# MaxInGaussian/SCFGP

Hardware: AMD Instinct MI355X
Metric: NLML+grad evals/sec (higher is better)
Workload: dtype f32

## Files before the change

scfgp_amd/csrc/apply.hip:

```cpp
#include "kernels.h"
#include "tile_cfgs.h"

#include <algorithm>

#ifdef SCFGP_TRACE
constexpr int ATRACE_CAP = 1 << 16;
__device__ unsigned long long g_atrace[5 * ATRACE_CAP][5];
int64_t apply_trace_read(void* host, int64_t max_bytes) {
    const int64_t n = max_bytes < (int64_t)sizeof(g_atrace) ? max_bytes : (int64_t)sizeof(g_atrace);
    return hipMemcpyFromSymbol(host, HIP_SYMBOL(g_atrace), n) == hipSuccess ? n : -2;
}
#else
int64_t apply_trace_read(void*, int64_t) { return -1; }
#endif
template <typename T, int TILE> struct ApplyCfg {
    typedef TileCfg<T, Tune<T>::APPLY_BM, TILE, SCFGP_BK, Tune<T>::APPLY_WGM, Tune<T>::apply_wgn(TILE), Tune<T>::MS,
                    SCFGP_BK == 16 && Tune<T>::MS == 16> type;
};

#include "apply_epilogue.h"

template <class Cfg, int EPI>
__device__ __forceinline__ void apply_tile(
    const typename Cfg::T* __restrict__ Phi, const typename Cfg::T* __restrict__ Bm, typename Cfg::T* V,
// ... 40 lines not shown
            __syncthreads();
            apply_tile<Cfg, EPI>(Phi, Bm, V, vpart, p, q, y, alpha, ut, K, Kp, Np, njt, col0, jt0, mu, ntot, o, rb, smem_raw);
        }
    } else
        apply_tile<Cfg, EPI>(Phi, Bm, V, vpart, p, q, y, alpha, ut, K, Kp, Np, njt, col0, jt0, mu, ntot, (int)(wid % njt), wid / njt, smem_raw);
}

typedef __attribute__((address_space(3))) void lds_void;
typedef const __attribute__((address_space(1))) void gbl_void;
template <typename T, int BN_>
struct ApplyDma {
    static constexpr int ES = (int)sizeof(T), BM = 256, BN = BN_, ROWB = 16 * ES, CPR = ROWB / 16;
    static constexpr int WN = ES == 4 ? 64 : 32;
    static constexpr int WAVES = 4 * (BN / WN), STAGE = (BM + BN) * ROWB, STAGES = 3, LDS_BYTES = STAGES * STAGE,
                         DMA_PER_WAVE = STAGE / 1024 / WAVES, ROWS_PER_DMA = 1024 / ROWB;
    static constexpr int PRE = 2;
    static constexpr int WAVES_PER_EU = WAVES == 4 ? 2 : 4;
    typedef TileCfg<T, BM, BN, 16, 4, BN / WN, 16, true> Cfg;
    static_assert(STAGE / 1024 % WAVES == 0 && LDS_BYTES <= 160 * 1024, "whole DMA instructions per wave; the ring fits the LDS");
    static __device__ __forceinline__ int swz(int x) {
        if constexpr (ES == 4) return (0x78 >> (2 * ((x >> 2) & 3))) & 3;
        else return (int)((0x6BEB08u >> (3 * ((x >> 1) & 7))) & 7);
    }
};
static_assert(((0x6BEB08u >> 0) & 7) == 0 && ((0x6BEB08u >> 3) & 7) == 1 && ((0x6BEB08u >> 6) & 7) == 4 && ((0x6BEB08u >> 9) & 7) == 5 &&
              ((0x6BEB08u >> 12) & 7) == 6 && ((0x6BEB08u >> 15) & 7) == 7 && ((0x6BEB08u >> 18) & 7) == 2 && ((0x6BEB08u >> 21) & 7) == 3,
              "fp64 swizzle table");

template <typename T, int EPI, int BN>
__global__ __launch_bounds__((64 * ApplyDma<T, BN>::WAVES)) __attribute__((amdgpu_waves_per_eu(ApplyDma<T, BN>::WAVES_PER_EU, ApplyDma<T, BN>::WAVES_PER_EU)))
void apply_dma_kernel(const T* __restrict__ Phi, const T* __restrict__ Bm, T* V,
                      double* __restrict__ vpart, const double* __restrict__ p, const double* __restrict__ q,
                      const double* __restrict__ y, const double* __restrict__ alpha, const double* __restrict__ ut,
                      int K, int Kp, int64_t Np, int njt, double* __restrict__ mu, int col0, int slot0, int64_t rb0) {
    typedef ApplyDma<T, BN> D;
    typedef typename D::Cfg Cfg;
    typedef T half_t __attribute__((ext_vector_type(2)));
    typedef std::integral_constant<int, 0> H0;
    typedef std::integral_constant<int, 1> H1;
    constexpr int DPW = D::DMA_PER_WAVE, NRD = Cfg::TM + Cfg::TN, NM = 2 * Cfg::TM * Cfg::TN, PRE = D::PRE;
    static_assert(Cfg::TM == 4 && (Cfg::TN == 4 || Cfg::TN == 2), "fragment lists of the wait statements");
    static_assert(PRE + DPW + NRD <= NM, "one fetch or read per MFMA behind the barrier");
    SMEM_DECL;
    char* smem = smem_raw;
#ifdef SCFGP_TRACE
    const unsigned long long tr_t0 = __builtin_amdgcn_s_memrealtime();
#endif
    const unsigned wid = xcd_remap(blockIdx.x, gridDim.x);
    const int jt = EPI == 3 || EPI == 4 ? (int)((wid % njt + wid / njt) % njt) : (int)(wid % njt);
    const int64_t rb = rb0 + wid / njt;
    const int cbase = col0 + jt * D::BN;
    const int lane = threadIdx.x & 63, wave = __builtin_amdgcn_readfirstlane(threadIdx.x >> 6);
    const char* src[DPW]; unsigned loff[DPW]; int dst[DPW];
#pragma unroll
    for (int u = 0; u < DPW; ++u) {
        const int t = wave * DPW + u, x0 = D::ROWS_PER_DMA * t, l = lane / D::CPR, c = (lane % D::CPR) ^ D::swz(x0 + l);
        const int xb = x0 - D::BM, xcol = (xb & ~(D::WN - 1)) + Cfg::TN * (xb & 15) + ((xb >> 4) & (Cfg::TN - 1));
        const T* rowp = x0 < D::BM ? Phi + (rb * D::BM + x0) * Kp : Bm + (int64_t)(cbase + xcol) * Kp;
        src[u] = reinterpret_cast<const char*>(rowp) + (EPI == 4 ? (cbase / 16) * D::ROWB : 0);
        loff[u] = (unsigned)((x0 < D::BM ? l : Cfg::TN * l) * Kp * D::ES + c * 16);
        dst[u] = t * 1024;
    }
    const auto fetch_one = [&](auto uc, int slot) {
        constexpr int u = decltype(uc)::value;
        __builtin_amdgcn_global_load_lds((gbl_void*)(src[u] + loff[u]), (lds_void*)(smem + slot * D::STAGE + dst[u]), 16, 0, 0);
        src[u] += D::ROWB;
    };
    const int i = lane & 15, qg = lane >> 4;
    const int wm0 = (wave / Cfg::WGN) * Cfg::WM, wn0 = (wave % Cfg::WGN) * Cfg::WN;
    const int hoff0 = sizeof(T) == 4 ? (((qg >> 1) ^ D::swz(i)) << 4) + 8 * (qg & 1) : ((2 * qg) ^ D::swz(i)) << 4;
    const int hoff1 = sizeof(T) == 4 ? (((2 + (qg >> 1)) ^ D::swz(i)) << 4) + 8 * (qg & 1) : ((2 * qg + 1) ^ D::swz(i)) << 4;
    const int ring = (int)(uintptr_t)smem, aoff = ring + (wm0 + i) * D::ROWB, boff = ring + D::BM * D::ROWB + (wn0 + i) * D::ROWB;
    const int ra[2] = {aoff + hoff0, aoff + hoff1}, rbb[2] = {boff + hoff0, boff + hoff1};
    half_t ha[2][Cfg::TM], hb[2][Cfg::TN];
    typename Cfg::MTr::acc_t acc[Cfg::TM][Cfg::TN];
    acc_zero<Cfg>(acc);
    const int nst_all = (K + 15) / 16, nst_tri = (cbase + D::BN + 15) / 16;
    const int nst = (EPI == 3 && nst_tri < nst_all ? nst_tri : nst_all) - (EPI == 4 ? cbase / 16 : 0);
#define SCFGP_LDS_READ(dst, addr, off)                                                                              \
    do {                                                                                                             \
        if constexpr (sizeof(T) == 4) asm volatile("ds_read_b64 %0, %1 offset:%2" : "=v"(dst) : "v"(addr), "n"(off));   \
// ... 118 lines not shown
template <typename T> struct ApplyPlan {
    static constexpr int NW = 2;
    int width[NW], count[NW], col0[NW], jt0[NW], total;
    explicit ApplyPlan(int K) {
        const int w[NW] = {128, 64};
        int col = 0, jt = 0;
        const bool small = K <= 256;
        for (int i = 0; i < NW; ++i) {
            width[i] = w[i];
            const bool last = i == NW - 1;
            count[i] = small && !last ? 0 : (last ? (K - col + w[i] - 1) / w[i] : (K - col) / w[i]);
            col0[i] = col; jt0[i] = jt;
            col += count[i] * w[i]; jt += count[i];
        }
        total = jt;
    }
};
bool F16x3Kernels::apply_runs(const Geom& g) { return ApplyPlan<float>(g.K).count[0] > 0; }
template <class Cfg, int EPI, typename T>
static int apply_launch_cfg(const Geom& g, int njt, int col0, int jt0, const T* Phi, const T* Bm, T* V, double* vpart,
                            const double* p, const double* q, const double* y, const double* alpha, const double* ut,
                            double* mu, int ntot, hipStream_t st) {
    if (njt <= 0) return 0;
    const int64_t nrb = g.Np / Cfg::BM;
    const int wgs_per_rb = EPI == 3 || EPI == 4 ? (njt + 1) / 2 : njt;
    allow_big_lds(apply_kernel<Cfg, EPI>, Cfg::LDS_BYTES);
    hipLaunchKernelGGL((apply_kernel<Cfg, EPI>), dim3((unsigned)(wgs_per_rb * nrb)), dim3(Cfg::THREADS), Cfg::LDS_BYTES, st,
                       Phi, Bm, V, vpart, p, q, y, alpha, ut, g.K, g.Kp, g.Np, njt, col0, jt0, mu, ntot);
    return (int)(njt * nrb);
}
template <typename T, int EPI, int BN>
static int apply_dma_launch(const Geom& g, int njt, int col0, int slot0, const T* Phi, const T* Bm, T* V, double* vpart,
                            const double* p, const double* q, const double* y, const double* alpha, const double* ut,
                            double* mu, hipStream_t st, int64_t rb0 = 0, int64_t nrb = -1) {
    typedef ApplyDma<T, BN> D;
    if (nrb < 0) nrb = g.Np / D::BM;
    if (njt <= 0 || nrb <= 0) return 0;
    allow_big_lds(apply_dma_kernel<T, EPI, BN>, D::LDS_BYTES);
    hipLaunchKernelGGL((apply_dma_kernel<T, EPI, BN>), dim3((unsigned)(njt * nrb)), dim3(64 * D::WAVES), D::LDS_BYTES, st,
                       Phi, Bm, V, vpart, p, q, y, alpha, ut, g.K, g.Kp, g.Np, njt, mu, col0, slot0, rb0);
    return (int)(njt * nrb);
}
static int apply_num_cus() {
    static int n = 0;
    if (n == 0) {
        int dev = 0; hipDeviceProp_t prop;
        if (hipGetDevice(&dev) == hipSuccess && hipGetDeviceProperties(&prop, dev) == hipSuccess) n = prop.multiProcessorCount;
        if (n <= 0) n = 256;
    }
    return n;
}
template <typename T, int EPI>
static int apply_launch(const Geom& g, const T* Phi, const T* Bm, T* V, double* vpart, const double* p, const double* q,
                        const double* y, const double* alpha, const double* ut, double* mu, hipStream_t st,
                        int dma = 0, const T* BmT = nullptr, const F16Operands* f16 = nullptr) {
    if (!BmT) BmT = Bm;
    const ApplyPlan<T> pl(g.K);
    int nb = 0;
    if constexpr (EPI != 2) {
        if (dma && pl.count[0] > 0) {
            int n256 = 0;
            const int64_t nrb = g.Np / 256;
            int64_t tail_rb = 0;
            if constexpr (sizeof(T) == 4) {
                n256 = dma == 2 ? pl.count[0] / 2 : 0;
                if (n256 > 0 && EPI != 3 && EPI != 4) {
                    const int64_t ncu = apply_num_cus(), tiles = nrb * n256, rem = tiles % ncu;
                    if (tiles > ncu && rem > 0 && 20 * rem <= 9 * ncu) tail_rb = (rem + n256 - 1) / n256;
                }
                if (f16 && (EPI == 0 || EPI == 1)) {
                    constexpr int E = EPI == 1 ? 1 : 0;
                    nb += F16x3Kernels::apply<E, 256>(g, n256, 0, 0, Phi, *f16, V, vpart, p, q, y, alpha, ut, mu, st, 0, nrb - tail_rb);
                    nb += F16x3Kernels::apply<E, 128>(g, pl.count[0] - 2 * n256, 256 * n256, 2 * n256, Phi, *f16, V, vpart, p, q, y, alpha, ut, mu, st, 0, nrb - tail_rb);
                    nb += F16x3Kernels::apply<E, 64>(g, pl.count[1], pl.col0[1], pl.jt0[1], Phi, *f16, V, vpart, p, q, y, alpha, ut, mu, st, 0, nrb - tail_rb);
                    if (tail_rb > 0) {
                        nb += F16x3Kernels::apply<E, 128>(g, pl.count[0], 0, 0, Phi, *f16, V, vpart, p, q, y, alpha, ut, mu, st, nrb - tail_rb, tail_rb);
                        nb += F16x3Kernels::apply<E, 64>(g, pl.count[1], pl.col0[1], pl.jt0[1], Phi, *f16, V, vpart, p, q, y, alpha, ut, mu, st, nrb - tail_rb, tail_rb);
                    }
                    return nb;
                }
                nb += apply_dma_launch<T, EPI, 256>(g, n256, 0, 0, Phi, BmT, V, vpart, p, q, y, alpha, ut, mu, st, 0, nrb - tail_rb);
            }
            nb += apply_dma_launch<T, EPI, 128>(g, pl.count[0] - 2 * n256, 256 * n256, 2 * n256, Phi, BmT, V, vpart, p, q, y, alpha, ut, mu, st, 0, nrb - tail_rb);
            nb += apply_dma_launch<T, EPI, 64>(g, pl.count[1], pl.col0[1], pl.jt0[1], Phi, BmT, V, vpart, p, q, y, alpha, ut, mu, st, 0, nrb - tail_rb);
            if (tail_rb > 0) {
                nb += apply_dma_launch<T, EPI, 128>(g, pl.count[0], 0, 0, Phi, BmT, V, vpart, p, q, y, alpha, ut, mu, st, nrb - tail_rb, tail_rb);
                nb += apply_dma_launch<T, EPI, 64>(g, pl.count[1], pl.col0[1], pl.jt0[1], Phi, BmT, V, vpart, p, q, y, alpha, ut, mu, st, nrb - tail_rb, tail_rb);
            }
            return nb;
        }
    }
    nb += apply_launch_cfg<typename ApplyCfg<T, 128>::type, EPI, T>(g, pl.count[0], pl.col0[0], pl.jt0[0], Phi, Bm, V, vpart, p, q, y, alpha, ut, mu, pl.total, st);
    nb += apply_launch_cfg<typename ApplyCfg<T, 64>::type, EPI, T>(g, pl.count[1], pl.col0[1], pl.jt0[1], Phi, Bm, V, vpart, p, q, y, alpha, ut, mu, pl.total, st);
    return nb;
}

template <typename T>
void ApplyKernels<T>::apply_v(const Geom& g, const T* Phi, const T* Bm, T* V, double* vpart, const double* alpha, double* mu,
                              hipStream_t st, int dma, const F16Operands* f16) {
    apply_launch<T, 0>(g, Phi, Bm, V, vpart, nullptr, nullptr, nullptr, alpha, nullptr, mu, st, dma, nullptr, f16);
}
template <typename T>
void ApplyKernels<T>::apply_predict(const Geom& g, const T* Phi, const T* LiT, double* vpart, const double* alpha, double* mu,
                                    hipStream_t st) {
    apply_launch<T, 2>(g, Phi, LiT, (T*)nullptr, vpart, nullptr, nullptr, nullptr, alpha, nullptr, mu, st);
}
template <typename T>
void ApplyKernels<T>::apply_plain(const Geom& g, const T* A, const T* Bm, T* Out, int Kc, int ncols, hipStream_t st) {
    Geom gk = g; gk.K = Kc;
    apply_launch_cfg<typename ApplyCfg<T, 64>::type, 4, T>(gk, (ncols + 63) / 64, 0, 0, A, Bm, Out, nullptr, nullptr, nullptr, nullptr, nullptr,
                                                           nullptr, nullptr, ApplyPlan<T>(Kc).total, st);
}

template <typename T>
void ApplyKernels<T>::apply_c(const Geom& g, const T* Phi, const T* LiT, const T* Li, T* C, double* vpart, const double* alpha,
                              const double* beta, double* mu, hipStream_t st, int dma) {
    const bool by_dma = dma && ApplyPlan<T>(g.K).count[0] > 0;
    apply_launch<T, 3>(g, Phi, LiT, C, vpart, nullptr, nullptr, nullptr, by_dma ? beta : alpha, nullptr, mu, st, dma, Li);
}
template <typename T>
void ApplyKernels<T>::apply_vc(const Geom& g, const T* C, const T* Li, const T* LiT, T* V, hipStream_t st, int dma) {
    apply_launch<T, 4>(g, C, Li, V, nullptr, nullptr, nullptr, nullptr, nullptr, nullptr, nullptr, st, dma, LiT);
}
template <typename T>
void ApplyKernels<T>::apply_phibar(const Geom& g, const T* Phi, const T* Abar, T* V, const double* p, const double* q,
                                   const double* y, const double* alpha, const double* ut, hipStream_t st, int dma, const F16Operands* f16) {
    apply_launch<T, 1>(g, Phi, Abar, V, nullptr, p, q, y, alpha, ut, nullptr, st, dma, nullptr, f16);
}

template <typename T> static int apply_njt(const Geom& g) { return ApplyPlan<T>(g.K).total; }


template <int MODE>
__global__ __launch_bounds__(256) void rowstats_kernel(const double* __restrict__ mupart, const double* __restrict__ vpart, int njt,
                                                       const double* __restrict__ y, const Scal* __restrict__ sc,
                                                       double* __restrict__ o1, double* __restrict__ o2,
                                                       double* __restrict__ partial, int64_t N, int64_t Np) {
    __shared__ double red[4][256];
    const double kappa = sc->kappa;
    double t2 = 0, kb = 0, qv = 0, pm = 0;
    for (int64_t n = (int64_t)blockIdx.x * 256 + threadIdx.x; n < Np; n += (int64_t)gridDim.x * 256) {
        double v = 0, mu = 0;
        for (int t = 0; t < njt; ++t) { v += vpart[(int64_t)t * Np + n]; mu += mupart[(int64_t)t * Np + n]; }
        const double d = kappa * (v + 1.0);
        if (MODE == 0) {
            double pn = 0, qn = 0;
            if (n < N) {
                const double r = mu - y[n];
                const double rv = r * r + v;
                const double e = 1.0 / d - rv / (d * d);
                pn = 2.0 * r / d;
                qn = 1.0 / d + kappa * e;
                t2 += rv / d + log(2.0 * M_PI * d);
                kb += e * (v + 1.0);
                qv += qn * v; pm += pn * mu;
            }
            o1[n] = pn; o2[n] = qn;
        } else if (n < N) {
            o1[n] = mu; o2[n] = sqrt(d);
        }
    }
    if (MODE == 0) {
        red[0][threadIdx.x] = t2; red[1][threadIdx.x] = kb; red[2][threadIdx.x] = qv; red[3][threadIdx.x] = pm;
        __syncthreads();
        for (int w = 128; w >= 1; w >>= 1) {
            if ((int)threadIdx.x < w)
                for (int k = 0; k < 4; ++k) red[k][threadIdx.x] += red[k][threadIdx.x + w];
            __syncthreads();
        }
        if (threadIdx.x < 4) partial[blockIdx.x * 4 + threadIdx.x] = red[threadIdx.x][0];
    }
}

template <typename T>
void ApplyKernels<T>::rowstats(const Geom& g, const double* mupart, const double* vpart, const double* y,
                               const Scal* sc, double* p, double* q, double* partial, int nblocks, hipStream_t st) {
    hipLaunchKernelGGL((rowstats_kernel<0>), dim3(nblocks), dim3(256), 0, st, mupart, vpart, apply_njt<T>(g), y, sc, p, q,
                       partial, g.N, g.Np);
}

template <typename T>
void ApplyKernels<T>::rowpredict(const Geom& g, const double* mupart, const double* vpart, const Scal* sc, double* mu, double* sd,
                                 hipStream_t st) {
    const int nblocks = (int)((g.Np + 255) / 256 < 1024 ? (g.Np + 255) / 256 : 1024);
    hipLaunchKernelGGL((rowstats_kernel<1>), dim3(nblocks), dim3(256), 0, st, mupart, vpart, apply_njt<T>(g),
                       (const double*)nullptr, sc, mu, sd, (double*)nullptr, g.N, g.Np);
}
template <typename T> int ApplyKernels<T>::partials(const Geom& g) { return apply_njt<T>(g); }
__global__ __launch_bounds__(256) void rowresidual_kernel(const double* __restrict__ mupart, int njt, const double* __restrict__ y,
                                                          double* __restrict__ r, int64_t N, int64_t Np) {
    for (int64_t n = (int64_t)blockIdx.x * 256 + threadIdx.x; n < Np; n += (int64_t)gridDim.x * 256) {
        double mu = 0;
        for (int t = 0; t < njt; ++t) mu += mupart[(int64_t)t * Np + n];
        r[n] = n < N ? y[n] - mu : 0.0;
    }
}
template <typename T>
void ApplyKernels<T>::rowresidual(const Geom& g, const double* mupart, const double* y, double* r, hipStream_t st) {
    const int nblocks = (int)((g.Np + 255) / 256 < 1024 ? (g.Np + 255) / 256 : 1024);
    hipLaunchKernelGGL(rowresidual_kernel, dim3(nblocks), dim3(256), 0, st, mupart, apply_njt<T>(g), y, r, g.N, g.Np);
}
template struct ApplyKernels<double>;
template struct ApplyKernels<float>;

__global__ __launch_bounds__(256) void reduce_scalars_kernel(const double* __restrict__ partial, int nblocks, int width,
                                                             double* __restrict__ scalars, int slot0) {
    __shared__ double red[256];
    for (int k = 0; k < width; ++k) {
        double s = 0;
        for (int b = threadIdx.x; b < nblocks; b += 256) s += partial[(int64_t)b * width + k];
        red[threadIdx.x] = s;
        __syncthreads();
        for (int m = 128; m >= 1; m >>= 1) {
            if (threadIdx.x < m) red[threadIdx.x] += red[threadIdx.x + m];
            __syncthreads();
        }
        if (threadIdx.x == 0) scalars[slot0 + k] = red[0];
        __syncthreads();
// ... 55 lines not shown
```

scfgp_amd/csrc/apply_f16.hip:

```cpp
#include "apply_epilogue.h"

typedef _Float16 h8 __attribute__((ext_vector_type(8)));
typedef _Float16 h4 __attribute__((ext_vector_type(4)));
typedef _Float16 h2 __attribute__((ext_vector_type(2)));
typedef __attribute__((address_space(3))) void lds_void;
typedef const __attribute__((address_space(1))) void gbl_void;

namespace {
constexpr int BM = 256, ROW = 128;
template <int BN_> struct F16Tile {
    static constexpr int BN = BN_, WAVES = 4 * (BN / 64), STAGE = (BM + BN) * ROW, STAGES = 2, LDS_BYTES = STAGES * STAGE,
                         DPW = STAGE / 1024 / WAVES, WAVES_PER_EU = WAVES == 16 ? 4 : 2;
    static_assert(STAGE / 1024 % WAVES == 0 && LDS_BYTES <= 160 * 1024, "whole DMA instructions per wave; the ring fits the LDS");
    typedef TileCfg<float, BM, BN, 16, 4, BN / 64, 16, true> Cfg;
};
__device__ __forceinline__ int swz8(int x) { return (int)((0x6BEB08u >> (3 * ((x >> 1) & 7))) & 7); }
template <int OFF> __device__ __forceinline__ void lds_read(h8& out, unsigned addr) {
    asm volatile("ds_read_b128 %0, %1 offset:%2" : "=v"(out) : "v"(addr), "n"(OFF));
}
#define SCFGP_F16_WAIT(n, x) asm volatile("s_waitcnt lgkmcnt(" #n ")" : "+v"(x[0]), "+v"(x[1]), "+v"(x[2]), "+v"(x[3]) :: "memory")
}

template <int EPI, int BN>
__global__ __launch_bounds__((64 * F16Tile<BN>::WAVES))
__attribute__((amdgpu_waves_per_eu(F16Tile<BN>::WAVES_PER_EU, F16Tile<BN>::WAVES_PER_EU)))
void apply_f16_kernel(const float* __restrict__ Phi, const unsigned* __restrict__ Phi16, const char* __restrict__ B16, const float* __restrict__ scale,
                      unsigned* __restrict__ V16, const float* __restrict__ vbound, float* V, double* __restrict__ vpart, const double* __restrict__ p, const double* __restrict__ q,
                      const double* __restrict__ y, const double* __restrict__ alpha, const double* __restrict__ ut,
                      int K, int Kp, int64_t Np, int njt, double* __restrict__ mu, int col0, int slot0, int64_t rb0) {
    typedef F16Tile<BN> D;
    typedef typename D::Cfg Cfg;
    constexpr int DPW = D::DPW, STAGE = D::STAGE;
    SMEM_DECL;
    char* smem = smem_raw;
    const unsigned wid = xcd_remap(blockIdx.x, gridDim.x);
    const int jt = wid % njt;
    const int64_t rb = rb0 + wid / njt;
    const int cbase = col0 + jt * BN;
    const int lane = threadIdx.x & 63, wave = __builtin_amdgcn_readfirstlane(threadIdx.x >> 6);
    const char* src[DPW]; int dst[DPW];
#pragma unroll
    for (int u = 0; u < DPW; ++u) {
        const int t = DPW * wave + u, x = 8 * t + lane / 8;
        if (x < BM) {
            src[u] = reinterpret_cast<const char*>(Phi16 + (rb * BM + x) * Kp) + (((lane % 8) ^ swz8(x)) << 4);
        } else {
            const int xb = x - BM, xcol = (xb & ~63) + 4 * (xb & 15) + ((xb >> 4) & 3);
            src[u] = B16 + (int64_t)(cbase + xcol) * Kp * 4 + (((lane % 8) ^ swz8(xb)) << 4);
        }
        dst[u] = t * 1024;
    }
    const auto fetch = [&](int slot) {
#pragma unroll
        for (int u = 0; u < DPW; ++u) {
            __builtin_amdgcn_global_load_lds((gbl_void*)src[u], (lds_void*)(smem + slot * STAGE + dst[u]), 16, 0, 0);
            src[u] += ROW;
        }
    };
    const int i = lane & 15, qg = lane >> 4;
    const int wm0 = (wave / Cfg::WGN) * Cfg::WM, wn0 = (wave % Cfg::WGN) * Cfg::WN;
    const int ch = 4 * (qg >> 1) + (qg & 1), sw = swz8(i);
    const unsigned lds0 = (unsigned)(uintptr_t)smem;
    const unsigned oah = (wm0 + i) * ROW + ((ch ^ sw) << 4), oal = (wm0 + i) * ROW + (((ch + 2) ^ sw) << 4);
    const unsigned obh = (BM + wn0 + i) * ROW + ((ch ^ sw) << 4), obl = (BM + wn0 + i) * ROW + (((ch + 2) ^ sw) << 4);
    typename Cfg::MTr::acc_t acc[Cfg::TM][Cfg::TN];
    acc_zero<Cfg>(acc);
    const int nst = (K + 31) / 32;
    fetch(0);
// ... 87 lines not shown
    }
    r1[threadIdx.x] = m;
    __syncthreads();
    for (int w = 128; w >= 1; w >>= 1) {
        if ((int)threadIdx.x < w) r1[threadIdx.x] = fmax(r1[threadIdx.x], r1[threadIdx.x + w]);
        __syncthreads();
    }
    if (threadIdx.x == 0) part[blockIdx.x] = r1[0];
}
__global__ __launch_bounds__(256) void split_operand_kernel(const double* __restrict__ M, int K, int Kp, const double* __restrict__ part, int nparts,
                                                            const Scal* __restrict__ sc, char* __restrict__ out, float* __restrict__ scale) {
    double m = 0;
    for (int b = 0; b < nparts; ++b) m = fmax(m, part[b]);
    const int em = m > 0 ? 14 - ilogb(m) : 0, ephi = 14 - ilogbf((float)sc->s);
    if (blockIdx.x == 0 && threadIdx.x == 0) { scale[0] = ldexpf(1.0f, -(em + ephi)); scale[1] = ldexpf(1.0f, em); }
    const int64_t total = (int64_t)Kp * Kp;
    for (int64_t e = (int64_t)blockIdx.x * 256 + threadIdx.x; e < total; e += (int64_t)gridDim.x * 256) {
        const int j = (int)(e / Kp), k = (int)(e % Kp);
        const double x = j < K && k < K ? ldexp(M[(int64_t)k * Kp + j], em) : 0.0;
        const _Float16 h = (_Float16)x, l = (_Float16)(x - (double)h);
        _Float16* row = reinterpret_cast<_Float16*>(out + (int64_t)j * Kp * 4 + (int64_t)(k / 16) * 64) + k % 16;
        row[0] = h; row[16] = l;
    }
}

void F16x3Kernels::split_operand(const Geom& g, const double* M, char* B16, float* scale, double* part, const Scal* sc, hipStream_t st) {
    constexpr int NP = 512;
    hipLaunchKernelGGL(maxabs_kernel, dim3(NP), dim3(256), 0, st, M, g.K, g.Kp, part);
    hipLaunchKernelGGL(split_operand_kernel, dim3(2048), dim3(256), 0, st, M, g.K, g.Kp, (const double*)part, NP, sc, B16, scale);
}
template <int EPI, int BN>
int F16x3Kernels::apply(const Geom& g, int njt, int col0, int slot0, const float* Phi, const F16Operands& f, float* V,
                        double* vpart, const double* p, const double* q, const double* y, const double* alpha, const double* ut, double* mu,
                        hipStream_t st, int64_t rb0, int64_t nrb) {
    typedef F16Tile<BN> D;
    if (njt <= 0 || nrb <= 0) return 0;
    allow_big_lds(apply_f16_kernel<EPI, BN>, D::LDS_BYTES);
    hipLaunchKernelGGL((apply_f16_kernel<EPI, BN>), dim3((unsigned)(njt * nrb)), dim3(64 * D::WAVES), D::LDS_BYTES, st,
                       Phi, f.Phi16, f.B16, f.scale, f.V16, f.vbound, V, vpart, p, q, y, alpha, ut, g.K, g.Kp, g.Np, njt, mu, col0, slot0, rb0);
    return (int)(njt * nrb);
}
#define SCFGP_F16_INST(EPI, BN)                                                                                                                       \
    template int F16x3Kernels::apply<EPI, BN>(const Geom&, int, int, int, const float*, const F16Operands&, float*, double*, const double*,          \
                                              const double*, const double*, const double*, const double*, double*, hipStream_t, int64_t, int64_t)
SCFGP_F16_INST(0, 256); SCFGP_F16_INST(1, 256); SCFGP_F16_INST(0, 128); SCFGP_F16_INST(1, 128); SCFGP_F16_INST(0, 64); SCFGP_F16_INST(1, 64);
#undef SCFGP_F16_INST
```

scfgp_amd/csrc/kernels.h:

```cpp
#pragma once
#include "common.h"

struct Geom {
    int D, S, M, J, K, P;
    int Dp;
    int Jp;
    int Sp;
    int lowrank;
    int Kp;
    int tile;
    int gfull;
    int gstrip;
    int64_t N;
    int64_t Np;
};

struct RowSplits {
    int nsplit;
    int groups;
    int units;
    int taper;
    int gran;
    int64_t nrb;
    __host__ __device__ int per_group() const { return units + taper; }
// ... 9 lines not shown
            e0 = base + den - (den >> k);
            e1 = k == taper ? base + den : base + den - (den >> (k + 1));
        }
        r0 = (g0 + len * e0 / (den * units)) * gran;
        r1 = (g0 + len * e1 / (den * units)) * gran;
    }
};
RowSplits gram_row_splits(int jobs_per_split, int64_t Np, bool f32, int nsplit_override, int taper);

struct Projection { const double* Fall; const double* Lall; const double* Rall; double* Tt; };

template <typename T>
struct FmapKernels {
    static void featuremap(const Geom& g, const double* Xt, const Projection& pr, const Scal* sc, T* Phi, hipStream_t st);
    static void convert(const double* src, T* dst, int K, int Kp, hipStream_t st);
    static void convert_transposed(const double* src, T* dst, int K, int Kp, hipStream_t st);
};

template <typename T>
struct GramKernels {
    static void gram(const Geom& g, const T* Phi, const double* w, const double* side, const RowSplits& rs, int64_t chunk,
                     double* slabs, double* sidepart, int* qhead, float* ws2, hipStream_t st);
    static int gram_jobs(const Geom& g);
    static void xtz(const Geom& g, const double* Xt, const T* Phi, const T* Phibar, int nsplit, int64_t chunk, double* slabs,
                    hipStream_t st);
    static void zbar_inplace(const Geom& g, const T* Phi, T* Phibar, hipStream_t st);
    static void rsel(const Geom& g, const double* params, T* out, hipStream_t st);
    static void tn_plain(const double* A, int Dp, const T* Bm, int64_t ldb, int J, int64_t Np, int nsplit, int64_t chunk, double* slabs,
                         hipStream_t st);
};

struct F16Operands { const unsigned* Phi16; const char* B16; const float* scale; unsigned* V16; const float* vbound; };

template <typename T>
struct ApplyKernels {
    static void apply_v(const Geom& g, const T* Phi, const T* Bm, T* V, double* vpart, const double* alpha, double* mupart,
                        hipStream_t st, int dma = 0, const F16Operands* f16 = nullptr);
    static void apply_predict(const Geom& g, const T* Phi, const T* LiT, double* vpart, const double* alpha, double* mupart,
                              hipStream_t st);
    static void apply_c(const Geom& g, const T* Phi, const T* LiT, const T* Li, T* C, double* vpart, const double* alpha,
                        const double* beta, double* mupart, hipStream_t st, int dma = 0);
    static void apply_vc(const Geom& g, const T* C, const T* Li, const T* LiT, T* V, hipStream_t st, int dma = 0);
    static void apply_phibar(const Geom& g, const T* Phi, const T* Abar, T* V, const double* p, const double* q,
                             const double* y, const double* alpha, const double* ut, hipStream_t st, int dma = 0, const F16Operands* f16 = nullptr);
    static void apply_plain(const Geom& g, const T* A, const T* Bm, T* Out, int Kc, int ncols, hipStream_t st);
    static void rowstats(const Geom& g, const double* mupart, const double* vpart, const double* y,
                         const Scal* sc, double* p, double* q, double* partial, int nblocks, hipStream_t st);
    static void rowpredict(const Geom& g, const double* mupart, const double* vpart, const Scal* sc, double* mu, double* sd,
                           hipStream_t st);
    static void rowresidual(const Geom& g, const double* mupart, const double* y, double* r, hipStream_t st);
    static int partials(const Geom& g);
};

struct F16x3Kernels {
    static void split_operand(const Geom& g, const double* M, char* B16, float* scale, double* part, const Scal* sc, hipStream_t st);
    template <int EPI, int BN>
    static int apply(const Geom& g, int njt, int col0, int slot0, const float* Phi, const F16Operands& f, float* V,
                     double* vpart, const double* p, const double* q, const double* y, const double* alpha, const double* ut, double* mu,
                     hipStream_t st, int64_t rb0, int64_t nrb);
    static bool apply_runs(const Geom& g);
    static constexpr size_t F16_PAD = 1024;
    static int side_blocks(const Geom& g);
    static void split_phi(const Geom& g, const float* Phi, const double* y, const Scal* sc, unsigned* Phi16, double* sidepart, float* tmp,
                          hipStream_t st);
    static void v_bound(const Geom& g, const double* B, const Scal* sc, float* tmp, hipStream_t st);
    static void split_v(const Geom& g, const float* V, const double* q, const double* p, unsigned* V16g, unsigned* qV16g, double* sidepart,
                        float* tmp, hipStream_t st);
    static int gram_chunks(const Geom& g, int64_t chunk);
    static int gram_tiles(const Geom& g);
    static void gram(const Geom& g, const unsigned* A16g, const unsigned* B16g, const float* scale, int64_t chunk, double* slabs, hipStream_t st);
};

template <typename T> struct SweepKernels : FmapKernels<T>, GramKernels<T>, ApplyKernels<T> {};

int64_t trace_read(void* host, int64_t max_bytes);
int64_t apply_trace_read(void* host, int64_t max_bytes);
int64_t chol_trace_read(void* host, int64_t max_bytes);

void reduce_tri_tiles(const double* slabs, int nsplit, int nts, int tile, double* packed, hipStream_t st);
void unpack_tri_tiles(const double* packed, int nts, int tile, double* full, int64_t ld, hipStream_t st);
void reduce_full_tiles(const double* slabs, int nsplit, int ntm, int ntn, double* out, int64_t ldo, hipStream_t st);
void reduce_side(const double* sidepart, int nsplit, int Kp, int ncov, double* vec, hipStream_t st);
void reduce_scalars(double* partial, int nblocks, int width, double* scalars, int slot0, hipStream_t st);
void sum_squares(const double* y, int64_t n, double* scalars, int slot, double* scratch, hipStream_t st);

void unpack_params(const Geom& g, const double* params, double* F, double* Fall, double* Lall, double* Rall, Scal* sc, hipStream_t st);
void grad_epilogue(const Geom& g, const double* params, const double* F, const double* XZ, int64_t ldxz,
                   double* work, double* scalars, int64_t Nglobal, double* grad, hipStream_t st,
                   const double* TZ = nullptr, int64_t ldtz = 0, const double* XU = nullptr, int64_t ldxu = 0);
void finalize_cost(const Geom& g, const Scal* sc, double* scalars, const double* yy, const double* t2kb,
                   int64_t Nglobal, double* grad, int want_grad, hipStream_t st);
void write_status(double* xs, double ran1, double cap1, double cap2, double fail, hipStream_t st);
// ... 125 lines not shown
```

scfgp_amd/csrc/scfgp_api.hip:

```cpp
#include "../../include/scfgp_hip.h"
#include "kernels.h"

#include <dlfcn.h>
#if __has_include(<rccl/rccl.h>)
#include <rccl/rccl.h>
#else
extern "C" {
typedef struct ncclComm* ncclComm_t;
typedef struct { char internal[128]; } ncclUniqueId;
typedef enum { ncclSuccess = 0 } ncclResult_t;
typedef enum { ncclFloat64 = 8 } ncclDataType_t;
typedef enum { ncclSum = 0 } ncclRedOp_t;
ncclResult_t ncclGetUniqueId(ncclUniqueId*);
ncclResult_t ncclCommInitRank(ncclComm_t*, int, ncclUniqueId, int);
ncclResult_t ncclAllReduce(const void*, void*, size_t, ncclDataType_t, ncclRedOp_t, ncclComm_t, hipStream_t);
ncclResult_t ncclCommDestroy(ncclComm_t);
const char* ncclGetErrorString(ncclResult_t);
}
#endif

#include <algorithm>
#include <cmath>
#include <cstdlib>
#include <cstring>
// ... 497 lines not shown
        const Geom& g = c->g;
        { ProfScope ps(c, "kstage_factor");
          hipMemcpyAsync(c->d_x1 + (int64_t)g.Kp * g.Kp, c->d_xp1 + c->n_pk, sizeof(double) * (g.Kp + 8), hipMemcpyDeviceToDevice, c->st);
          kstage_factor(c->kstage(), c->d_xp1, c->d_sc, c->st); }
        if (c->last_cform) {
            SK::convert(c->d_Li, (T*)c->d_BT, g.K, g.Kp, c->st);
            SK::convert_transposed(c->d_Li, (T*)c->d_AbarT, g.K, g.Kp, c->st);
        } else {
            SK::convert(c->d_B, (T*)c->d_BT, g.K, g.Kp, c->st);
            if (c->f16_on()) {
                F16x3Kernels::split_operand(g, c->d_B, c->d_B16, c->d_f16scale, c->d_partial, c->d_sc, c->st);
                F16x3Kernels::v_bound(g, c->d_B, c->d_sc, c->d_f16tmp, c->st);
            }
        }
        HIPCHK(c, hipGetLastError());
        return SCFGP_OK;
    }
    static int pass2(scfgp_ctx* c, int want_grad) {
        const Geom& g = c->g;
        if (c->last_cform) {
            const int dma = c->dma() ? 1 : 0;
            { ProfScope ps(c, "apply_c");
              SK::apply_c(g, (const T*)c->d_Phi, (const T*)c->d_AbarT, (const T*)c->d_BT, (T*)c->d_C, c->d_vpart, c->alpha(), c->beta(), c->d_mu, c->st, dma); }
            { ProfScope ps(c, "apply_vc");
              SK::apply_vc(g, (const T*)c->d_C, (const T*)c->d_BT, (const T*)c->d_AbarT, (T*)c->d_V, c->st, dma); }
        } else {
            ProfScope ps(c, "apply_v");
            F16Operands f16 = c->f16ops();
            if (want_grad && c->f16_gram()) f16.V16 = c->d_V16g;
            SK::apply_v(g, (const T*)c->d_Phi, (const T*)c->d_BT, (T*)c->d_V, c->d_vpart, c->alpha(), c->d_mu, c->st, c->dma(), c->f16_on() ? &f16 : nullptr);
        }
        const int nb = (int)std::min<int64_t>(g.Np / 4, 2048);
        { ProfScope ps(c, "rowstats");
          SK::rowstats(g, c->d_mu, c->d_vpart, c->d_y, c->d_sc, c->d_p, c->d_q, c->d_partial, nb, c->st);
          reduce_scalars(c->d_partial, nb, 4, c->xs2(), 0, c->st);
          write_status(c->xs2(), 0.0, 0.0, 0.0, 0.0, c->st); }
        if (want_grad) {
            gram_to(c, c->last_cform ? (const T*)c->d_C : (const T*)c->d_V, c->d_q, c->d_p, c->d_xp2, "gram_w");
        }
        HIPCHK(c, hipGetLastError());
        return SCFGP_OK;
    }
    static int adjoint(scfgp_ctx* c) {
        const Geom& g = c->g;
        { ProfScope ps(c, "kstage_adjoint"); unpack_exchange(c, c->d_xp2, c->d_x2);
          if (c->last_cform) kstage_adjoint_factor_form(c->kstage(), c->d_x2, c->d_Abar, c->d_sc, c->st);
          else kstage_adjoint(c->kstage(), c->d_x2, c->d_Abar, c->d_sc, c->st);
          kstage_bbar(c->kstage(), c->d_xp1, c->d_Abar, c->d_partial, c->st); }
        SK::convert(c->d_Abar, (T*)c->d_AbarT, g.K, g.Kp, c->st);
        if (c->f16_on()) F16x3Kernels::split_operand(g, c->d_Abar, c->d_B16, c->d_f16scale, c->d_partial, c->d_sc, c->st);
        HIPCHK(c, hipGetLastError());
        return SCFGP_OK;
    }
    static int pass3(scfgp_ctx* c) {
        const Geom& g = c->g;
        { ProfScope ps(c, "apply_phibar");
          const F16Operands f16 = c->f16ops();
          SK::apply_phibar(g, (const T*)c->d_Phi, (const T*)c->d_AbarT, (T*)c->d_V, c->d_p, c->d_q, c->d_y, c->alpha(), c->ut(), c->st, c->dma(),
                           c->f16_on() ? &f16 : nullptr);
          write_status(c->x3_scalars(), 0.0, 0.0, 0.0, 0.0, c->st); }
        const int ntm = c->Dpp / XT, ntn = g.Jp / XT;
        const int64_t chunk = c->dtype == SCFGP_F32 ? c->gram_chunk : 0;
        c->last_lrb = c->want_lrb();
        if (c->last_lrb) {
            ProfScope ps(c, "xtz");
            T* Zb = (T*)c->d_V; T* U = (T*)c->d_V + g.Jp;
            SK::zbar_inplace(g, (const T*)c->d_Phi, Zb, c->st);
// ... 2073 lines not shown
```

Measured before the change: 4.865.

## Fold the tail row-block apply into the BN=64 launch as a second region

Result: no change. 4.875, median of 5 (+0.2%).

```diff
diff --git a/scfgp_amd/csrc/apply.hip b/scfgp_amd/csrc/apply.hip
--- a/scfgp_amd/csrc/apply.hip
+++ b/scfgp_amd/csrc/apply.hip
@@ -96,7 +96,7 @@
 void apply_dma_kernel(const T* __restrict__ Phi, const T* __restrict__ Bm, T* V,
                       double* __restrict__ vpart, const double* __restrict__ p, const double* __restrict__ q,
                       const double* __restrict__ y, const double* __restrict__ alpha, const double* __restrict__ ut,
-                      int K, int Kp, int64_t Np, int njt, double* __restrict__ mu, int col0, int slot0, int64_t rb0) {
+                      int K, int Kp, int64_t Np, int njt, double* __restrict__ mu, int col0, int slot0, int64_t rb0, ApplyRegion rest) {
     typedef ApplyDma<T, BN> D;
     typedef typename D::Cfg Cfg;
     typedef T half_t __attribute__((ext_vector_type(2)));
@@ -110,7 +110,10 @@
 #ifdef SCFGP_TRACE
     const unsigned long long tr_t0 = __builtin_amdgcn_s_memrealtime();
 #endif
-    const unsigned wid = xcd_remap(blockIdx.x, gridDim.x);
+    unsigned wid = xcd_remap(blockIdx.x, gridDim.x);
+    if constexpr (BN == 64) {
+        if (wid >= rest.n_a) { wid -= rest.n_a; njt = rest.njt; col0 = rest.col0; slot0 = rest.slot0; rb0 = rest.rb0; }
+    }
     const int jt = EPI == 3 || EPI == 4 ? (int)((wid % njt + wid / njt) % njt) : (int)(wid % njt);
     const int64_t rb = rb0 + wid / njt;
     const int cbase = col0 + jt * D::BN;
@@ -295,14 +298,16 @@
 template <typename T, int EPI, int BN>
 static int apply_dma_launch(const Geom& g, int njt, int col0, int slot0, const T* Phi, const T* Bm, T* V, double* vpart,
                             const double* p, const double* q, const double* y, const double* alpha, const double* ut,
-                            double* mu, hipStream_t st, int64_t rb0 = 0, int64_t nrb = -1) {
+                            double* mu, hipStream_t st, int64_t rb0 = 0, int64_t nrb = -1, int njt_b = 0, int64_t nrb_b = 0) {
     typedef ApplyDma<T, BN> D;
     if (nrb < 0) nrb = g.Np / D::BM;
-    if (njt <= 0 || nrb <= 0) return 0;
+    const int64_t n_a = njt > 0 && nrb > 0 ? njt * nrb : 0, n_b = BN == 64 && njt_b > 0 && nrb_b > 0 ? njt_b * nrb_b : 0;
+    if (n_a + n_b <= 0) return 0;
+    const ApplyRegion rest{(unsigned)n_a, njt_b, 0, 0, rb0 + (nrb > 0 ? nrb : 0)};
     allow_big_lds(apply_dma_kernel<T, EPI, BN>, D::LDS_BYTES);
-    hipLaunchKernelGGL((apply_dma_kernel<T, EPI, BN>), dim3((unsigned)(njt * nrb)), dim3(64 * D::WAVES), D::LDS_BYTES, st,
-                       Phi, Bm, V, vpart, p, q, y, alpha, ut, g.K, g.Kp, g.Np, njt, mu, col0, slot0, rb0);
-    return (int)(njt * nrb);
+    hipLaunchKernelGGL((apply_dma_kernel<T, EPI, BN>), dim3((unsigned)(n_a + n_b)), dim3(64 * D::WAVES), D::LDS_BYTES, st,
+                       Phi, Bm, V, vpart, p, q, y, alpha, ut, g.K, g.Kp, g.Np, njt, mu, col0, slot0, rb0, rest);
+    return (int)(n_a + n_b);
 }
 static int apply_num_cus() {
     static int n = 0;
@@ -312,6 +317,12 @@
         if (n <= 0) n = 256;
     }
     return n;
+}
+template <typename T> static int64_t apply_tail_rb(const Geom& g, int dma, bool tri) {
+    const ApplyPlan<T> pl(g.K);
+    if (sizeof(T) != 4 || dma != 2 || tri || pl.count[0] < 2) return 0;
+    const int64_t n256 = pl.count[0] / 2, ncu = apply_num_cus(), tiles = g.Np / 256 * n256, rem = tiles % ncu;
+    return tiles > ncu && rem > 0 && 20 * rem <= 9 * ncu ? (rem + n256 - 1) / n256 : 0;
 }
 template <typename T, int EPI>
 static int apply_launch(const Geom& g, const T* Phi, const T* Bm, T* V, double* vpart, const double* p, const double* q,
@@ -324,32 +335,23 @@
         if (dma && pl.count[0] > 0) {
             int n256 = 0;
             const int64_t nrb = g.Np / 256;
-            int64_t tail_rb = 0;
+            const int64_t tail_rb = apply_tail_rb<T>(g, dma, EPI == 3 || EPI == 4);
+            const int njt_b = tail_rb > 0 ? (g.K + 63) / 64 : 0;
             if constexpr (sizeof(T) == 4) {
                 n256 = dma == 2 ? pl.count[0] / 2 : 0;
-                if (n256 > 0 && EPI != 3 && EPI != 4) {
-                    const int64_t ncu = apply_num_cus(), tiles = nrb * n256, rem = tiles % ncu;
-                    if (tiles > ncu && rem > 0 && 20 * rem <= 9 * ncu) tail_rb = (rem + n256 - 1) / n256;
-                }
                 if (f16 && (EPI == 0 || EPI == 1)) {
                     constexpr int E = EPI == 1 ? 1 : 0;
                     nb += F16x3Kernels::apply<E, 256>(g, n256, 0, 0, Phi, *f16, V, vpart, p, q, y, alpha, ut, mu, st, 0, nrb - tail_rb);
                     nb += F16x3Kernels::apply<E, 128>(g, pl.count[0] - 2 * n256, 256 * n256, 2 * n256, Phi, *f16, V, vpart, p, q, y, alpha, ut, mu, st, 0, nrb - tail_rb);
-                    nb += F16x3Kernels::apply<E, 64>(g, pl.count[1], pl.col0[1], pl.jt0[1], Phi, *f16, V, vpart, p, q, y, alpha, ut, mu, st, 0, nrb - tail_rb);
-                    if (tail_rb > 0) {
-                        nb += F16x3Kernels::apply<E, 128>(g, pl.count[0], 0, 0, Phi, *f16, V, vpart, p, q, y, alpha, ut, mu, st, nrb - tail_rb, tail_rb);
-                        nb += F16x3Kernels::apply<E, 64>(g, pl.count[1], pl.col0[1], pl.jt0[1], Phi, *f16, V, vpart, p, q, y, alpha, ut, mu, st, nrb - tail_rb, tail_rb);
-                    }
+                    nb += F16x3Kernels::apply<E, 64>(g, pl.count[1], pl.col0[1], pl.jt0[1], Phi, *f16, V, vpart, p, q, y, alpha, ut, mu, st, 0, nrb - tail_rb,
+                                                     njt_b, tail_rb);
                     return nb;
                 }
                 nb += apply_dma_launch<T, EPI, 256>(g, n256, 0, 0, Phi, BmT, V, vpart, p, q, y, alpha, ut, mu, st, 0, nrb - tail_rb);
             }
             nb += apply_dma_launch<T, EPI, 128>(g, pl.count[0] - 2 * n256, 256 * n256, 2 * n256, Phi, BmT, V, vpart, p, q, y, alpha, ut, mu, st, 0, nrb - tail_rb);
-            nb += apply_dma_launch<T, EPI, 64>(g, pl.count[1], pl.col0[1], pl.jt0[1], Phi, BmT, V, vpart, p, q, y, alpha, ut, mu, st, 0, nrb - tail_rb);
-            if (tail_rb > 0) {
-                nb += apply_dma_launch<T, EPI, 128>(g, pl.count[0], 0, 0, Phi, BmT, V, vpart, p, q, y, alpha, ut, mu, st, nrb - tail_rb, tail_rb);
-                nb += apply_dma_launch<T, EPI, 64>(g, pl.count[1], pl.col0[1], pl.jt0[1], Phi, BmT, V, vpart, p, q, y, alpha, ut, mu, st, nrb - tail_rb, tail_rb);
-            }
+            nb += apply_dma_launch<T, EPI, 64>(g, pl.count[1], pl.col0[1], pl.jt0[1], Phi, BmT, V, vpart, p, q, y, alpha, ut, mu, st, 0, nrb - tail_rb,
+                                               njt_b, tail_rb);
             return nb;
         }
     }
@@ -396,6 +398,7 @@
 
 template <int MODE>
 __global__ __launch_bounds__(256) void rowstats_kernel(const double* __restrict__ mupart, const double* __restrict__ vpart, int njt,
+                                                       int64_t n_b, int njt_b,
                                                        const double* __restrict__ y, const Scal* __restrict__ sc,
                                                        double* __restrict__ o1, double* __restrict__ o2,
                                                        double* __restrict__ partial, int64_t N, int64_t Np) {
@@ -404,7 +407,8 @@
     double t2 = 0, kb = 0, qv = 0, pm = 0;
     for (int64_t n = (int64_t)blockIdx.x * 256 + threadIdx.x; n < Np; n += (int64_t)gridDim.x * 256) {
         double v = 0, mu = 0;
-        for (int t = 0; t < njt; ++t) { v += vpart[(int64_t)t * Np + n]; mu += mupart[(int64_t)t * Np + n]; }
+        const int nt = n >= n_b ? njt_b : njt;
+        for (int t = 0; t < nt; ++t) { v += vpart[(int64_t)t * Np + n]; mu += mupart[(int64_t)t * Np + n]; }
         const double d = kappa * (v + 1.0);
         if (MODE == 0) {
             double pn = 0, qn = 0;
@@ -437,16 +441,17 @@
 
 template <typename T>
 void ApplyKernels<T>::rowstats(const Geom& g, const double* mupart, const double* vpart, const double* y,
-                               const Scal* sc, double* p, double* q, double* partial, int nblocks, hipStream_t st) {
-    hipLaunchKernelGGL((rowstats_kernel<0>), dim3(nblocks), dim3(256), 0, st, mupart, vpart, apply_njt<T>(g), y, sc, p, q,
-                       partial, g.N, g.Np);
+                               const Scal* sc, double* p, double* q, double* partial, int nblocks, hipStream_t st, int dma) {
+    const int64_t tail_rb = apply_tail_rb<T>(g, dma, false);
+    hipLaunchKernelGGL((rowstats_kernel<0>), dim3(nblocks), dim3(256), 0, st, mupart, vpart, apply_njt<T>(g),
+                       g.Np - 256 * tail_rb, tail_rb > 0 ? (g.K + 63) / 64 : 0, y, sc, p, q, partial, g.N, g.Np);
 }
 
 template <typename T>
 void ApplyKernels<T>::rowpredict(const Geom& g, const double* mupart, const double* vpart, const Scal* sc, double* mu, double* sd,
                                  hipStream_t st) {
     const int nblocks = (int)((g.Np + 255) / 256 < 1024 ? (g.Np + 255) / 256 : 1024);
-    hipLaunchKernelGGL((rowstats_kernel<1>), dim3(nblocks), dim3(256), 0, st, mupart, vpart, apply_njt<T>(g),
+    hipLaunchKernelGGL((rowstats_kernel<1>), dim3(nblocks), dim3(256), 0, st, mupart, vpart, apply_njt<T>(g), g.Np, 0,
                        (const double*)nullptr, sc, mu, sd, (double*)nullptr, g.N, g.Np);
 }
 template <typename T> int ApplyKernels<T>::partials(const Geom& g) { return apply_njt<T>(g); }
diff --git a/scfgp_amd/csrc/apply_f16.hip b/scfgp_amd/csrc/apply_f16.hip
--- a/scfgp_amd/csrc/apply_f16.hip
+++ b/scfgp_amd/csrc/apply_f16.hip
@@ -27,13 +27,16 @@
 void apply_f16_kernel(const float* __restrict__ Phi, const unsigned* __restrict__ Phi16, const char* __restrict__ B16, const float* __restrict__ scale,
                       unsigned* __restrict__ V16, const float* __restrict__ vbound, float* V, double* __restrict__ vpart, const double* __restrict__ p, const double* __restrict__ q,
                       const double* __restrict__ y, const double* __restrict__ alpha, const double* __restrict__ ut,
-                      int K, int Kp, int64_t Np, int njt, double* __restrict__ mu, int col0, int slot0, int64_t rb0) {
+                      int K, int Kp, int64_t Np, int njt, double* __restrict__ mu, int col0, int slot0, int64_t rb0, ApplyRegion rest) {
     typedef F16Tile<BN> D;
     typedef typename D::Cfg Cfg;
     constexpr int DPW = D::DPW, STAGE = D::STAGE;
     SMEM_DECL;
     char* smem = smem_raw;
-    const unsigned wid = xcd_remap(blockIdx.x, gridDim.x);
+    unsigned wid = xcd_remap(blockIdx.x, gridDim.x);
+    if constexpr (BN == 64) {
+        if (wid >= rest.n_a) { wid -= rest.n_a; njt = rest.njt; col0 = rest.col0; slot0 = rest.slot0; rb0 = rest.rb0; }
+    }
     const int jt = wid % njt;
     const int64_t rb = rb0 + wid / njt;
     const int cbase = col0 + jt * BN;
@@ -187,16 +190,18 @@
 template <int EPI, int BN>
 int F16x3Kernels::apply(const Geom& g, int njt, int col0, int slot0, const float* Phi, const F16Operands& f, float* V,
                         double* vpart, const double* p, const double* q, const double* y, const double* alpha, const double* ut, double* mu,
-                        hipStream_t st, int64_t rb0, int64_t nrb) {
+                        hipStream_t st, int64_t rb0, int64_t nrb, int njt_b, int64_t nrb_b) {
     typedef F16Tile<BN> D;
-    if (njt <= 0 || nrb <= 0) return 0;
+    const int64_t n_a = njt > 0 && nrb > 0 ? njt * nrb : 0, n_b = BN == 64 && njt_b > 0 && nrb_b > 0 ? njt_b * nrb_b : 0;
+    if (n_a + n_b <= 0) return 0;
+    const ApplyRegion rest{(unsigned)n_a, njt_b, 0, 0, rb0 + (nrb > 0 ? nrb : 0)};
     allow_big_lds(apply_f16_kernel<EPI, BN>, D::LDS_BYTES);
-    hipLaunchKernelGGL((apply_f16_kernel<EPI, BN>), dim3((unsigned)(njt * nrb)), dim3(64 * D::WAVES), D::LDS_BYTES, st,
-                       Phi, f.Phi16, f.B16, f.scale, f.V16, f.vbound, V, vpart, p, q, y, alpha, ut, g.K, g.Kp, g.Np, njt, mu, col0, slot0, rb0);
-    return (int)(njt * nrb);
+    hipLaunchKernelGGL((apply_f16_kernel<EPI, BN>), dim3((unsigned)(n_a + n_b)), dim3(64 * D::WAVES), D::LDS_BYTES, st,
+                       Phi, f.Phi16, f.B16, f.scale, f.V16, f.vbound, V, vpart, p, q, y, alpha, ut, g.K, g.Kp, g.Np, njt, mu, col0, slot0, rb0, rest);
+    return (int)(n_a + n_b);
 }
 #define SCFGP_F16_INST(EPI, BN)                                                                                                                       \
     template int F16x3Kernels::apply<EPI, BN>(const Geom&, int, int, int, const float*, const F16Operands&, float*, double*, const double*,          \
-                                              const double*, const double*, const double*, const double*, double*, hipStream_t, int64_t, int64_t)
+                                              const double*, const double*, const double*, const double*, double*, hipStream_t, int64_t, int64_t, int, int64_t)
 SCFGP_F16_INST(0, 256); SCFGP_F16_INST(1, 256); SCFGP_F16_INST(0, 128); SCFGP_F16_INST(1, 128); SCFGP_F16_INST(0, 64); SCFGP_F16_INST(1, 64);
 #undef SCFGP_F16_INST
diff --git a/scfgp_amd/csrc/kernels.h b/scfgp_amd/csrc/kernels.h
--- a/scfgp_amd/csrc/kernels.h
+++ b/scfgp_amd/csrc/kernels.h
@@ -65,6 +65,7 @@
 
 struct F16Operands { const unsigned* Phi16; const char* B16; const float* scale; unsigned* V16; const float* vbound; };
 
+struct ApplyRegion { unsigned n_a; int njt, col0, slot0; int64_t rb0; };
 template <typename T>
 struct ApplyKernels {
     static void apply_v(const Geom& g, const T* Phi, const T* Bm, T* V, double* vpart, const double* alpha, double* mupart,
@@ -78,7 +79,7 @@
                              const double* y, const double* alpha, const double* ut, hipStream_t st, int dma = 0, const F16Operands* f16 = nullptr);
     static void apply_plain(const Geom& g, const T* A, const T* Bm, T* Out, int Kc, int ncols, hipStream_t st);
     static void rowstats(const Geom& g, const double* mupart, const double* vpart, const double* y,
-                         const Scal* sc, double* p, double* q, double* partial, int nblocks, hipStream_t st);
+                         const Scal* sc, double* p, double* q, double* partial, int nblocks, hipStream_t st, int dma = 0);
     static void rowpredict(const Geom& g, const double* mupart, const double* vpart, const Scal* sc, double* mu, double* sd,
                            hipStream_t st);
     static void rowresidual(const Geom& g, const double* mupart, const double* y, double* r, hipStream_t st);
@@ -90,7 +91,7 @@
     template <int EPI, int BN>
     static int apply(const Geom& g, int njt, int col0, int slot0, const float* Phi, const F16Operands& f, float* V,
                      double* vpart, const double* p, const double* q, const double* y, const double* alpha, const double* ut, double* mu,
-                     hipStream_t st, int64_t rb0, int64_t nrb);
+                     hipStream_t st, int64_t rb0, int64_t nrb, int njt_b = 0, int64_t nrb_b = 0);
     static bool apply_runs(const Geom& g);
     static constexpr size_t F16_PAD = 1024;
     static int side_blocks(const Geom& g);
diff --git a/scfgp_amd/csrc/scfgp_api.hip b/scfgp_amd/csrc/scfgp_api.hip
--- a/scfgp_amd/csrc/scfgp_api.hip
+++ b/scfgp_amd/csrc/scfgp_api.hip
@@ -553,7 +553,7 @@
         }
         const int nb = (int)std::min<int64_t>(g.Np / 4, 2048);
         { ProfScope ps(c, "rowstats");
-          SK::rowstats(g, c->d_mu, c->d_vpart, c->d_y, c->d_sc, c->d_p, c->d_q, c->d_partial, nb, c->st);
+          SK::rowstats(g, c->d_mu, c->d_vpart, c->d_y, c->d_sc, c->d_p, c->d_q, c->d_partial, nb, c->st, c->last_cform ? 0 : c->dma());
           reduce_scalars(c->d_partial, nb, 4, c->xs2(), 0, c->st);
           write_status(c->xs2(), 0.0, 0.0, 0.0, 0.0, c->st); }
         if (want_grad) {
```
